# iqbal-lab-org/make_prg

Hardware: AMD Instinct MI355X
Metric: MSAs/sec (from_msa, whole node) on 30k-gene pan-genome (higher is better)
Workload: dtype u8 (+f64 KMeans)

## Files before the change

make_prg_amd/csrc/k_cluster.inc:

```
#define CF_TILE 256
#define CF_TILE_BIG 32
#define CF_ROWS 1024
static_assert(CF_TILE == MPRG_CF_TILE && CF_TILE_BIG == MPRG_CF_TILE_BIG && CF_ROWS == MPRG_CF_ROWS, "include/mprg.h documents the tiles");
MPRG_DEV long long cf_col_tiles(long long n_cols, long long n_rows) {
  const long long tw = n_rows > CF_ROWS ? CF_TILE_BIG : CF_TILE;
  return (n_cols + tw - 1) / tw;
}
#ifndef CFH_WIDE
#define CFH_WIDE MPRG_CF_WIDE
#endif
#define CFH_G 16
#define CFH_ROWS_WIDE 16
static_assert(CFH_ROWS_WIDE == MPRG_CF_ROWS_WIDE, "include/mprg.h documents the chunks");
MPRG_DEV int cf_chunk_rows(long long n_cols, long long n_rows) { return (n_cols >= CFH_WIDE && n_rows > CF_ROWS) ? CFH_ROWS_WIDE : CF_TILE; }
MPRG_DEV long long cf_row_chunks(long long n_cols, long long n_rows) { const int ch = cf_chunk_rows(n_cols, n_rows); return (n_rows + ch - 1) / ch; }
#define CFO_THREADS 128
#define CFO_POOL 8192
MPRG_DEV long long cf_lds_bytes(long long S, long long n, long long k) {
  const long long cp = (n + 3) & ~3LL;
  return ((S + 3) & ~3LL) + ((2 * S + 3) & ~3LL) + k * cp + S * cp;
}
MPRG_DEV bool cf_one_fits(long long S, long long n, long long k) { return S >= 1 && S < 65536 && n >= 1 && cf_lds_bytes(S, n, k) <= CFO_POOL; }
#ifndef CF_THREADS
#define CF_THREADS 128
#endif
KERNEL(k_cluster_majority, const uint8_t *arena, const int64_t *views, const int32_t *rowidx, const int64_t *prob_all,
       const int32_t *work, int k, const int32_t *d_of_row_all, const int32_t *labels_all, int32_t *assign_all,
       const double *km_info, int32_t *scratch_all, const uint8_t *gcodes_all, const int32_t *kinfo, int one_form, DsCount dc) {
  DS_GUARD(dc, 1);
  const int32_t *wk = work + 2 * (long long)BLOCK_ID;
  if (kinfo && kinfo[5 * (long long)wk[0] + 1] == 0) return;
  const int64_t *P = prob_all + (long long)wk[0] * PF;
  const ViewD d = load_view(views, (int)P[0]);
  if (one_form && cf_one_fits(d.n_rows, d.n_cols, k)) return;
  const int n = d.n_cols, S = d.n_rows, D = (int)P[1], tile = S > CF_ROWS ? CF_TILE_BIG : CF_TILE, c0 = wk[1] * tile;
  const int32_t *dor = d_of_row_all + d.row_off;
  const int32_t *labels = labels_all ? labels_all + P[10] : nullptr;
  uint8_t *maj = (uint8_t *)(scratch_all + d.col_off * 3);
  SHARED(uint32_t, cnt, 12 * CF_THREADS);
  SHARED(int32_t, first, 12 * CF_THREADS);
  if (wk[1] == 0 && labels && assign_all && (!km_info || km_info[8 * (long long)wk[0] + 3] >= (double)k)) {
    PAR_FOR(q, D) { assign_all[P[10] + q] = labels[q]; }
  }
  if (S > CF_ROWS) return;
  SHARED(int32_t, mrk, 2 * CF_ROWS);
  int32_t *mrow = mrk, *mkey = mrk + CF_ROWS;
  SHARED(int, coff, 16);
  SHARED(int, cfill, 16);
  PAR_FOR(q, 16) { coff[q] = 0; }
  BARRIER();
  PAR_FOR(i, S) {
    const int dd = dor[i];
    if (dd < 0) continue;
    const int cl = labels ? labels[dd] : 0;
    if (cl >= 0 && cl < k) ATOMIC_ADD(coff + cl + 1, 1);
  }
  BARRIER();
  ONE_THREAD { for (int q = 1; q <= k; ++q) coff[q] += coff[q - 1]; for (int q = 0; q < k; ++q) cfill[q] = coff[q]; }
  BARRIER();
  PAR_FOR(i, S) {
    const int dd = dor[i];
    if (dd < 0) continue;
    const int cl = labels ? labels[dd] : 0;
    if (cl < 0 || cl >= k) continue;
    const int pos = ATOMIC_ADD(cfill + cl, 1);
    mrow[pos] = gcodes_all ? (int)i : view_row(d, rowidx, i);
    mkey[pos] = dd * S + i;
  }
  BARRIER();
#define CF_COUNT(x, key) do { if ((x) < 12) { cnt[(x) * CF_THREADS + t] += 1; if ((key) < first[(x) * CF_THREADS + t]) first[(x) * CF_THREADS + t] = (key); } } while (0)
  const int ncols = n - c0 < tile ? n - c0 : tile;
  const int n_items = k * ncols;
  int slices = n_items <= N_THREADS ? N_THREADS / n_items : 1;
  if (slices > 8) slices = 8;
  for (int item0 = 0; item0 < n_items; item0 += N_THREADS) {
    const int t = (int)threadIdx.x;
    const int item = item0 + (slices > 1 ? t % n_items : t), sl = slices > 1 ? t / n_items : 0;
    const bool live = item < n_items && sl < slices;
    const int cl = live ? (int)((unsigned)item / (unsigned)ncols) : 0, c = c0 + (live ? (int)((unsigned)item % (unsigned)ncols) : 0);
    if (live) {
      for (int s = 0; s < 12; ++s) { cnt[s * CF_THREADS + t] = 0; first[s * CF_THREADS + t] = 0x7fffffff; }
      const uint8_t *col = gcodes_all ? gcodes_all + d.aux0 + c : arena + d.rm + d.col0 + c;
      const long long cpitch = gcodes_all ? u_pitch(n) : d.pitchC;
      const int lo = coff[cl], len = coff[cl + 1] - lo, per = (len + slices - 1) / slices;
      int m = lo + sl * per;
      const int m1 = lo + ((sl + 1) * per < len ? (sl + 1) * per : len);
      for (; m + 8 <= m1; m += 8) {
        unsigned x[8];
#pragma unroll
        for (int q = 0; q < 8; ++q) x[q] = col[(long long)mrow[m + q] * cpitch] & 15u;
#pragma unroll
        for (int q = 0; q < 8; ++q) CF_COUNT(x[q], mkey[m + q]);
      }
      for (; m < m1; ++m) { const unsigned x = col[(long long)mrow[m] * cpitch] & 15u; CF_COUNT(x, mkey[m]); }
    }
    if (slices > 1) BARRIER();
    if (live && sl == 0) {
      int best = 0; uint32_t best_n = 0; int32_t best_key = 0x7fffffff;
      for (int s = 0; s < 12; ++s) {
        uint32_t a = cnt[s * CF_THREADS + t]; int32_t key = first[s * CF_THREADS + t];
        for (int o = 1; o < slices; ++o) {
          a += cnt[s * CF_THREADS + t + o * n_items];
          const int32_t ko = first[s * CF_THREADS + t + o * n_items];
          if (ko < key) key = ko;
        }
        if (s == 0 || a > best_n || (a == best_n && key < best_key)) { best = s; best_n = a; best_key = key; }
      }
      maj[(long long)cl * n + c] = (uint8_t)best;
    }
  }
#undef CF_COUNT
}

#define CFB_THREADS 1024
KERNEL(k_cluster_majority_big, const uint8_t *arena, const int64_t *views, const int32_t *rowidx, const int64_t *prob_all,
       const int32_t *work, int k, const int32_t *d_of_row_all, const int32_t *labels_all, int32_t *scratch_all,
       const uint8_t *gcodes_all, const int32_t *kinfo, DsCount dc) {
  DS_GUARD(dc, 1);
  const int32_t *wk = work + 2 * (long long)BLOCK_ID;
  if (kinfo && kinfo[5 * (long long)wk[0] + 1] == 0) return;
  const int64_t *P = prob_all + (long long)wk[0] * PF;
  const ViewD d = load_view(views, (int)P[0]);
  const int n = d.n_cols, S = d.n_rows, c0 = wk[1] * CF_TILE_BIG;
  if (S <= CF_ROWS) return;
  const int32_t *dor = d_of_row_all + d.row_off;
  const int32_t *labels = labels_all ? labels_all + P[10] : nullptr;
  uint8_t *maj = (uint8_t *)(scratch_all + d.col_off * 3);
  __shared__ uint32_t cnt[KM_KMAX * CF_TILE_BIG * 12];
  __shared__ unsigned long long key[KM_KMAX * CF_TILE_BIG * 12];
  const int ncols = n - c0 < CF_TILE_BIG ? n - c0 : CF_TILE_BIG;
  PAR_FOR(e, k * CF_TILE_BIG * 12) { cnt[e] = 0; key[e] = ~0ULL; }
  BARRIER();
  const int t = (int)threadIdx.x, cg = t % (CF_TILE_BIG / 4), sl = t / (CF_TILE_BIG / 4), slices = N_THREADS / (CF_TILE_BIG / 4), cb = 4 * cg;
  if (cb < ncols && sl < slices) {
    const uint8_t *col = gcodes_all ? gcodes_all + d.aux0 + c0 + cb : arena + d.rm + d.col0 + c0 + cb;
    const long long cpitch = gcodes_all ? u_pitch(n) : d.pitchC;
    const int per = (S + slices - 1) / slices, i0 = sl * per, i1 = (sl + 1) * per < S ? (sl + 1) * per : S;
#define CFB_ROW(w_, dd_, i_, cl_) do {                                                                                                \
      const unsigned long long key_ = ((unsigned long long)(uint32_t)(dd_) << 32) | (uint32_t)(i_);                                   \
      _Pragma("unroll") for (int u_ = 0; u_ < 4; ++u_) {                                                                              \
        const unsigned x_ = ((w_) >> (8 * u_)) & 15u;                                                                                 \
        if (cb + u_ < ncols && x_ < 12) {                                                                                             \
          const int at_ = (((cl_) * CF_TILE_BIG + cb + u_) * 12) + (int)x_;                                                           \
          atomicAdd(&cnt[at_], 1u);                                                                                                   \
          if (key_ < key[at_]) atomicMin(&key[at_], key_);                                                                            \
        } } } while (0)
    int i = i0;
    for (; i + 8 <= i1; i += 8) {
      int dd8[8], lab8[8]; uint32_t w8[8];
#pragma unroll
      for (int q = 0; q < 8; ++q) dd8[q] = dor[i + q];
#pragma unroll
      for (int q = 0; q < 8; ++q) {
        lab8[q] = (labels && dd8[q] >= 0) ? labels[dd8[q]] : 0;
        __builtin_memcpy(&w8[q], col + (long long)(gcodes_all ? i + q : view_row(d, rowidx, i + q)) * cpitch, 4);
      }
#pragma unroll
      for (int q = 0; q < 8; ++q) if (dd8[q] >= 0 && lab8[q] >= 0 && lab8[q] < k) CFB_ROW(w8[q], dd8[q], i + q, lab8[q]);
    }
    for (; i < i1; ++i) {
      const int dd = dor[i];
      if (dd < 0) continue;
      const int cl = labels ? labels[dd] : 0;
      if (cl < 0 || cl >= k) continue;
// ... 175 lines not shown
```

make_prg_amd/csrc/k_kloop.inc:

```

#ifndef KL_CF_FN
#define KL_CF_FN MPRG_DEV
#endif
#ifdef MPRG_TEST_CF_GLOBAL
#define KL_CF_IN_LDS(fits) false
#else
#define KL_CF_IN_LDS(fits) (fits)
#endif
#define KL_CF_FIELD_BITS 32
MPRG_DEV int cf_row_cluster(int i, const uint8_t *mlab_s, const int32_t *dor, const int32_t *labels) {
  if (mlab_s) return mlab_s[i];
  const int dd = dor[i];
  return dd < 0 ? 255 : labels[dd];
}
template <int FB> struct CfWords {
  static constexpr int PER = 64 / FB, W = 12 / PER;
  unsigned long long w[W];
  MPRG_DEVM void clear() {
#pragma unroll
    for (int q = 0; q < W; ++q) w[q] = 0;
  }
  MPRG_DEVM void add(unsigned x) {
    const unsigned long long inc = x < 12 ? 1ull << (FB * (x % PER)) : 0ull;
    const unsigned sel = x / PER;
#pragma unroll
    for (int q = 0; q < W; ++q) w[q] += sel == (unsigned)q ? inc : 0ull;
  }
  MPRG_DEVM unsigned long long count(int s) const {
    return (w[s / PER] >> (FB * (s % PER))) & ((FB == 32) ? 0xffffffffull : 0xffffull);
  }
};
template <int FB, int POOLB>
KL_CF_FN bool cf_problem_fb(const int S, const int n, const int D, const int k, const int32_t *dor, const int32_t *labels, int32_t *assign,
                            uint8_t *maj, const uint8_t *G, uint8_t *pool, int *flag_s) {
  typedef CfWords<FB> Words;
  const int cpitch = u_pitch(n);
  const bool staged = S <= POOLB;
  uint8_t *mlab_w = staged ? pool : nullptr;
  const uint8_t *mlab_s = mlab_w;
  const int items = k * n;
  const long long acc_off = staged ? ((S + 7) & ~7) : 0;
  int slices = 1;
#ifndef KL_NO_SLICES
  if (items * 2 <= N_THREADS) {
    slices = N_THREADS / items; if (slices > 16) slices = 16;
    if (acc_off + (long long)items * slices * Words::W * 8 > POOLB) slices = 1;
  }
#endif
  unsigned long long *acc = (unsigned long long *)(pool + acc_off);
  PAR_FOR(q, D) { assign[q] = labels[q]; }
  if (staged) { PAR_FOR(i, S) { const int dd = dor[i]; mlab_w[i] = dd < 0 ? (uint8_t)255 : (uint8_t)labels[dd]; } }
  ONE_THREAD { flag_s[0] = 0; }
  BARRIER();
  for (int e0 = 0; e0 < items * slices; e0 += N_THREADS) {
    const int e = e0 + (int)threadIdx.x;
    const bool live = e < items * slices;
    const int item = live ? (slices > 1 ? e % items : e) : 0, sl = slices > 1 ? e / items : 0;
    const int cl = (int)((unsigned)item / (unsigned)n), c = (int)((unsigned)item % (unsigned)n);
    Words cw;
    cw.clear();
    const uint8_t *col = G + c;
    if (live) {
      const int per = (S + slices - 1) / slices;
      int i = sl * per;
      const int i1 = (sl + 1) * per < S ? (sl + 1) * per : S;
      for (; i + 4 <= i1; i += 4) {
        int rc[4]; unsigned x[4];
#pragma unroll
        for (int q = 0; q < 4; ++q) rc[q] = cf_row_cluster(i + q, mlab_s, dor, labels);
#pragma unroll
        for (int q = 0; q < 4; ++q) x[q] = rc[q] == cl ? (unsigned)col[(long long)(i + q) * cpitch] & 15u : 15u;
#pragma unroll
        for (int q = 0; q < 4; ++q) cw.add(x[q]);
      }
      for (; i < i1; ++i) if (cf_row_cluster(i, mlab_s, dor, labels) == cl) cw.add((unsigned)col[(long long)i * cpitch] & 15u);
      if (slices > 1 && sl > 0) {
#pragma unroll
        for (int q = 0; q < Words::W; ++q) acc[((long long)sl * items + item) * Words::W + q] = cw.w[q];
      }
    }
    if (slices > 1) {
      BARRIER();
      if (live && sl == 0) {
        for (int o = 1; o < slices; ++o)
#pragma unroll
          for (int q = 0; q < Words::W; ++q) cw.w[q] += acc[((long long)o * items + item) * Words::W + q];
      }
    }
    if (live && sl == 0) {
      unsigned long long best_n = 0;
#pragma unroll
      for (int s = 0; s < 12; ++s) { const unsigned long long a = cw.count(s); best_n = a > best_n ? a : best_n; }
      unsigned tied = 0;
#pragma unroll
      for (int s = 0; s < 12; ++s) if (cw.count(s) == best_n) tied |= 1u << s;
      int best = __ffs(tied) - 1;
      if (best_n > 0 && (tied & (tied - 1))) {
        long long best_key = 0x7fffffffffffffffLL;
#pragma nounroll
        for (int i = 0; i < S; ++i) {
          if (cf_row_cluster(i, mlab_s, dor, labels) != cl) continue;
          const unsigned x = (unsigned)col[(long long)i * cpitch] & 15u;
          if (!((tied >> x) & 1u)) continue;
          const long long key = (long long)dor[i] * S + i;
          if (key < best_key) { best_key = key; best = (int)x; }
        }
      }
      maj[(long long)cl * n + c] = (uint8_t)best;
    }
  }
  BARRIER();
  const int thresh = n < 5 ? 1 : (int)(0.2 * (double)n);
  PAR_FOR(i, S) {
    const int cl = cf_row_cluster((int)i, mlab_s, dor, labels);
    if (cl == 255) continue;
    const uint8_t *m = maj + (long long)cl * n;
    const uint8_t *grow = G + (long long)i * cpitch;
    int dist = 0;
#pragma nounroll
    for (int c = 0; c < n && dist <= thresh; c += 8) {
      uint64_t x, y;
      __builtin_memcpy(&x, grow + c, 8);
      __builtin_memcpy(&y, m + c, 8);
      uint64_t v = (x ^ y) & 0x0f0f0f0f0f0f0f0fULL;
      if (c + 8 > n) v &= 0xffffffffffffffffULL >> (8 * (c + 8 - n));
      const uint64_t nz = (((v & 0x7f7f7f7f7f7f7f7fULL) + 0x7f7f7f7f7f7f7f7fULL) | v) & 0x8080808080808080ULL;
      dist += __popcll(nz);
    }
    if (dist > thresh) flag_s[0] = 1;
  }
  BARRIER();
  const bool further = flag_s[0] != 0;
  BARRIER();
  return further;
}

template <bool OPT = false>
MPRG_DEV bool cf_problem_lds(const int S, const int n, const int D, const int k, const int32_t *dor, const int32_t *labels, int32_t *assign,
                             const uint8_t *G, uint8_t *pool, int *flag_s) {
  typedef CfWords<16> Words;
  const int cpitch = u_pitch(n), cp = (n + 3) & ~3, cw4 = cp >> 2;
  uint8_t *mlab = pool;
  uint16_t *dk = (uint16_t *)(pool + ((S + 3) & ~3));
  uint8_t *majs = (uint8_t *)dk + ((2 * S + 3) & ~3);
  uint8_t *cells = majs + k * cp;
  if (!OPT || assign) { PAR_FOR(q, D) { assign[q] = labels[q]; } }
  PAR_FOR(i, S) { const int dd = dor[i]; mlab[i] = dd < 0 ? (uint8_t)255 : ((OPT && !labels) ? (uint8_t)0 : (uint8_t)labels[dd]); dk[i] = (uint16_t)dd; }
  PAR_FOR(e, S * cw4) {
    const int i = (int)((unsigned)e / (unsigned)cw4), w = (int)((unsigned)e % (unsigned)cw4);
    *(uint32_t *)(cells + i * cp + 4 * w) = *(const uint32_t *)(G + (long long)i * cpitch + 4 * w) & 0x0f0f0f0fu;
  }
  ONE_THREAD { flag_s[0] = 0; }
  BARRIER();
  PAR_FOR(item, k * n) {
    const int cl = (int)((unsigned)item / (unsigned)n), c = (int)((unsigned)item % (unsigned)n);
    Words cw;
    cw.clear();
    const uint8_t *col = cells + c;
    int i = 0;
    for (; i + 4 <= S; i += 4) {
      unsigned rc[4], x[4];
#pragma unroll
      for (int q = 0; q < 4; ++q) { rc[q] = mlab[i + q]; x[q] = col[(i + q) * cp]; }
#pragma unroll
      for (int q = 0; q < 4; ++q) cw.add(rc[q] == (unsigned)cl ? x[q] : 15u);
    }
    for (; i < S; ++i) cw.add(mlab[i] == cl ? (unsigned)col[i * cp] : 15u);
    unsigned long long best_n = 0;
#pragma unroll
    for (int s_ = 0; s_ < 12; ++s_) { const unsigned long long a = cw.count(s_); best_n = a > best_n ? a : best_n; }
    unsigned tied = 0;
#pragma unroll
    for (int s_ = 0; s_ < 12; ++s_) if (cw.count(s_) == best_n) tied |= 1u << s_;
    int best = __ffs(tied) - 1;
    if (best_n > 0 && (tied & (tied - 1))) {
      int best_key = 0x7fffffff;
#pragma nounroll
      for (int r = 0; r < S; ++r) {
        const unsigned x = col[r * cp];
        if (mlab[r] != cl || !((tied >> x) & 1u)) continue;
        const int key = (int)dk[r] * S + r;
        if (key < best_key) { best_key = key; best = (int)x; }
      }
    }
    majs[cl * cp + c] = (uint8_t)best;
  }
  BARRIER();
  const int thresh = n < 5 ? 1 : (int)(0.2 * (double)n);
  PAR_FOR(i, S) {
    const int cl = mlab[i];
    if (cl == 255) continue;
    const uint8_t *m = majs + cl * cp, *row = cells + i * cp;
    int dist = 0;
#pragma nounroll
    for (int c = 0; c < n; c += 4) {
      uint32_t v = *(const uint32_t *)(row + c) ^ *(const uint32_t *)(m + c);
      if (c + 4 > n) v &= 0xffffffffu >> (8 * (c + 4 - n));
      const uint32_t nz = (((v & 0x7f7f7f7fu) + 0x7f7f7f7fu) | v) & 0x80808080u;
      dist += __popc(nz);
    }
    if (dist > thresh) flag_s[0] = 1;
  }
  BARRIER();
  const bool further = flag_s[0] != 0;
  BARRIER();
  return further;
}

struct KlUoff { int32_t v[KM_KMAX + 1]; };
enum { KL_ST_FITS = 80, KL_ST_BAD = 82, KL_ST_CF = 84, KL_ST_BYTES_GENERAL = 85, KL_ST_BYTES_SMALL = 93 };
template <int RMAX, int NEEDCAP, int LAB8, int POOLB, int KCH, int K_HI>
MPRG_DEV void kl_problem(const int b, const int64_t *prob_all, int n_init, const double *uniforms_all, const KlUoff &uoff,
                         const double *xcounts, double *ws_all, const int64_t *views, const int32_t *d_of_row_all,
                         const uint8_t *gcodes_all, int32_t *scratch_all, int32_t *labels_all, int32_t *assign_all, double *km_info,
                         int32_t *km_status, int32_t *num_clusters, int32_t *active, int64_t *stats, int bytes_slot, uint8_t *pool,
                         int sel_lab_cap) {
  SHARED(int32_t, ki_s, 8);
  SHARED(int, cf_flag, 1);
  SHARED(int, st_i, 4);
  SHARED(double, st_d, 2);
  ONE_THREAD { st_i[0] = num_clusters[b]; st_i[1] = 1; st_i[2] = 0; st_i[3] = 0; st_d[0] = 0; st_d[1] = 0; }
  BARRIER();
  for (;;) {
    const int k = st_i[0] + 1;
    const int D = (int)prob_all[(long long)b * PF + 1];
    BARRIER();
    if (k > KM_KMAX || k == D) { ONE_THREAD { st_i[0] = k; st_i[1] = 0; } break; }
    if (k > K_HI) break;
    ONE_THREAD { ki_s[0] = b; ki_s[1] = k; ki_s[2] = 0; ki_s[3] = uoff.v[k]; ki_s[4] = 0; km_status[b] = 0; }
    BARRIER();
    km_restarts_body<RMAX, NEEDCAP, LAB8, POOLB, KCH>(0, prob_all, ki_s, n_init, uniforms_all, xcounts, ws_all, nullptr, km_status + b, pool);
    BARRIER();
    KM_T0();
    km_select_body(0, prob_all, ki_s, n_init, xcounts, ws_all, nullptr, labels_all, km_info + 8 * (long long)b, (int32_t *)pool, sel_lab_cap);
    BARRIER(); KM_T(12);
    const int64_t *P = prob_all + (long long)b * PF;
    const double *info = km_info + 8 * (long long)b;
    const bool accepted = info[3] >= (double)k;
    const ViewD d = load_view(views, (int)P[0]);
    ONE_THREAD {
      st_i[2] += 1;
      st_d[0] += 8.0 * (double)P[1] * (double)P[7] * (info[4] + (double)n_init);
      if (km_status[b] & MPRG_KM_UNSUPPORTED) st_i[3] = 1;
      if (accepted) { st_i[0] = k; st_d[1] += (double)d.n_rows * (double)d.n_cols; }
      else st_i[1] = 0;
// ... 88 lines not shown
    BARRIER();
    KM_T0();
    const double *info = km_info + 8 * (long long)b;
    const bool accepted = info[3] >= (double)k;
    const ViewD d = load_view(views, (int)P[0]);
    ONE_THREAD {
      st_i[2] += 1;
      st_d[0] += 8.0 * (double)P[1] * (double)P[7] * (info[4] + (double)ki_s[5]);
      if (km_status[b] & MPRG_KM_UNSUPPORTED) st_i[3] = 1;
      if (accepted) { st_i[0] = k; st_d[1] += (double)d.n_rows * (double)d.n_cols; }
      else st_i[1] = 0;
    }
    if (!accepted) break;
    const int32_t *dor = d_of_row_all + d.row_off;
    int32_t *labels = labels_all + P[10], *assign = assign_all + P[10];
    uint8_t *maj = (uint8_t *)(scratch_all + d.col_off * 3);
    const uint8_t *G = gcodes_all + d.aux0;
    const bool cf_behind = KL_CF_IN_LDS(cf_lds_bytes(d.n_rows, d.n_cols, k) <= lds_size - head);
    const bool further = cf_behind ? cf_problem_lds(d.n_rows, d.n_cols, D, k, dor, labels, assign, G, pool + head, cf_flag)
                                   : cf_problem_fb<KL_CF_FIELD_BITS, KML_C0>(d.n_rows, d.n_cols, D, k, dor, labels, assign, maj, G, pool, cf_flag);
    if (!cf_behind) staged = false;
    KM_T(13);
    if (!further) { ONE_THREAD { st_i[1] = 0; } break; }
  }
  BARRIER();
  ONE_THREAD {
    num_clusters[b] = st_i[0]; active[b] = st_i[1];
    if (st_i[2]) {
      atomicAdd((unsigned long long *)stats + KL_ST_FITS, (unsigned long long)st_i[2]);
      atomicAdd((double *)stats + KL_ST_BYTES_SMALL, st_d[0]);
      if (st_d[1] != 0) atomicAdd((double *)stats + KL_ST_CF, st_d[1]);
      if (st_i[3]) stats[KL_ST_BAD] = 1;
    }
  }
}
__attribute__((amdgpu_flat_work_group_size(64, 1024), amdgpu_waves_per_eu(KM_WAVES, KM_WAVES))) __global__ void k_cluster_loop_lds(
    const int64_t *prob_all, int n_init, const double *uniforms_all, KlUoff uoff, const double *xcounts, double *ws_all,
    const int64_t *views, const int32_t *d_of_row_all, const uint8_t *gcodes_all, int32_t *scratch_all, int32_t *labels_all,
    int32_t *assign_all, double *km_info, int32_t *km_status, int32_t *num_clusters, int32_t *active, int64_t *stats, int cls, int lds_bytes,
    DsCount dc) {
  DS_GUARD(dc, 1);
  HIP_DYNAMIC_SHARED(uint8_t, pool)
  const int b = BLOCK_ID;
  if (!active[b]) return;
  const int64_t *P = prob_all + (long long)b * PF;
  const int c = kml_class_ws(P[1], P[7], num_clusters[b] + 1, n_init, true, ws_all + P[9]);
  if (c < 0 || c > cls) return;
  kll_problem(b, prob_all, n_init, uniforms_all, uoff, xcounts, ws_all, views, d_of_row_all, gcodes_all, scratch_all, labels_all, assign_all, km_info,
              km_status, num_clusters, active, stats, pool, lds_bytes, cls);
}

KERNEL(k_cluster_further_one, const int64_t *views, const int64_t *prob_all, int n_probs, int k, const int32_t *d_of_row_all,
       const int32_t *labels_all, int32_t *assign_all, const double *km_info, int32_t *out_further, const uint8_t *gcodes_all,
       const int32_t *kinfo, DsCount dc) {
  DS_GUARD(dc, 1);
  const int b = BLOCK_ID;
  if (kinfo && kinfo[5 * (long long)b + 1] == 0) return;
  const int64_t *P = prob_all + (long long)b * PF;
  const ViewD d = load_view(views, (int)P[0]);
  if (!cf_one_fits(d.n_rows, d.n_cols, k)) return;
  __shared__ __attribute__((aligned(16))) uint8_t pool[CFO_POOL];
  SHARED(int, flag, 1);
  const int32_t *labels = labels_all ? labels_all + P[10] : nullptr;
  int32_t *assign = (labels && assign_all && (!km_info || km_info[8 * (long long)b + 3] >= (double)k)) ? assign_all + P[10] : nullptr;
  const bool further = cf_problem_lds<true>(d.n_rows, d.n_cols, (int)P[1], k, d_of_row_all + d.row_off, labels, assign, gcodes_all + d.aux0, pool, flag);
  ONE_THREAD { out_further[b] = further ? 1 : 0; }
}
```

make_prg_amd/csrc/mprg_api.hip:

```cpp
#include "mprg_platform.h"
#include "../../include/mprg.h"
#include <stdio.h>
#include <initializer_list>
#include <string.h>

#include "k_ingest.inc"
#include "k_columns.inc"
#include "k_partition.inc"
#include "k_rows.inc"
#include "k_kmer.inc"
#include "k_kmeans.inc"
#include "k_kmeans_lds.inc"
#include "k_cluster.inc"
#include "k_kloop.inc"
#include "k_emit.inc"
#include "k_forest.inc"
#include "k_align.inc"
#include "k_star.inc"
#include "k_refine.inc"
#include "k_prog.inc"
#include "k_prog_band.inc"
#include "k_collapse.inc"
#include "host_encoders.inc"
#include "host_batch.inc"

static thread_local char g_err[512] = "";
static int fail(const char *what) { snprintf(g_err, sizeof g_err, "%s", what); return -1; }

static int check_launch(const char *name) {
  hipError_t e = hipGetLastError();
  if (e != hipSuccess) { snprintf(g_err, sizeof g_err, "%s: %s", name, hipGetErrorString(e)); return -2; }
  return 0;
}

#include "runtime_api.inc"

#define BLOCK_VIEW 256
#include <stdlib.h>
static int env_threads(const char *name, int dflt, int hi = 1024) {
  const char *e = getenv(name);
  const int v = e ? atoi(e) : dflt;
  return (v >= 64 && v <= hi && v % 64 == 0) ? v : dflt;
}
static const int g_pf_threads = env_threads("MPRG_PF_THREADS", BLOCK_VIEW);
static const int g_dd_threads = env_threads("MPRG_DD_THREADS", BLOCK_VIEW, 512);
static const int g_km_threads = env_threads("MPRG_KM_THREADS", 256);
static const int g_km_wide_threads = env_threads("MPRG_KM_WIDE_THREADS", 1024);
static const int g_kp_threads = env_threads("MPRG_KP_THREADS", 0);
static const int g_kp_tiled = [] { const char *e = getenv("MPRG_KP_TILED"); return (e && atoi(e) == 0) ? 0 : 1; }();
static const int g_kpw_split = [] { const char *e = getenv("MPRG_KPW_SPLIT"); return (e && atoi(e) == 0) ? 0 : 1; }();
static const int g_kms_threads = env_threads("MPRG_KMS_THREADS", 128, 128);
static const int g_kml_flags = [] { const char *e = getenv("MPRG_KML_FLAGS"); return e ? (atoi(e) & 0x7f) : 0; }();
static const int g_kml_threads[KML_CLASSES] = {env_threads("MPRG_KML_THREADS0", 128, 256), env_threads("MPRG_KML_THREADS1", 128, 256),
                                               env_threads("MPRG_KML_THREADS2", 256, 1024), env_threads("MPRG_KML_THREADS3", 256, 1024),
                                               env_threads("MPRG_KML_THREADS4", 512, 1024), env_threads("MPRG_KML_THREADS5", 1024, 1024)};
template <class K> static int kml_raise_lds(K kernel, bool *raised, const char *what) {
  if (*raised) return 0;
  if (hipFuncSetAttribute((const void *)kernel, hipFuncAttributeMaxDynamicSharedMemorySize, KML_C5) != hipSuccess) return fail(what);
  *raised = true;
  return 0;
}
static const int g_cf_one = [] { const char *e = getenv("MPRG_CF_ONE"); return (e && atoi(e) == 0) ? 0 : 1; }();
static const int g_pw_wave = [] { const char *e = getenv("MPRG_WAVE_VIEWS"); return (e && atoi(e) == 0) ? 0 : 1; }();
static const int g_row_views = [] { const char *e = getenv("MPRG_ROW_VIEWS"); return (e && atoi(e) == 0) ? 0 : 1; }();
#define RV_THREADS 128
#define RV_THREADS_S 64

extern "C" {

#ifndef MPRG_BUILD_TAG
#define MPRG_BUILD_TAG "hip gfx950"
#endif
const char *mprg_version(void) { return "mprg 0.2 (" MPRG_BUILD_TAG ")"; }
const char *mprg_last_error(void) { return g_err; }

int mprg_device_cus(void) {
  int dev = 0; hipDeviceProp_t p;
  if (hipGetDevice(&dev) != hipSuccess || hipGetDeviceProperties(&p, dev) != hipSuccess) return fail("no HIP device");
  return p.multiProcessorCount;
}

int mprg_ingest(const uint8_t *raw, const int64_t *msa_table, int n_msas, int64_t n_tiles, const uint8_t *n_replacement,
                uint8_t *arena, int64_t arena_bytes, int32_t *status, void *stream) {
  if (n_msas <= 0) return 0;
  if (hipMemsetAsync(arena, 15, (size_t)arena_bytes, (hipStream_t)stream) != hipSuccess) return fail("memset");
  if (hipMemsetAsync(status, 0, sizeof(int32_t) * n_msas, (hipStream_t)stream) != hipSuccess) return fail("memset");
  if (n_tiles > 0) LAUNCH(k_ingest, n_tiles, 256, stream, raw, msa_table, n_msas, n_replacement, arena, status);
  return check_launch("k_ingest");
}

int mprg_column_residue_counts(const uint8_t *raw, const int64_t *table, const int32_t *work, int n_work, int32_t *out,
                               void *stream) {
  if (n_work <= 0) return 0;
  LAUNCH(k_column_residue_counts, n_work, 256, stream, raw, table, work, out);
  return check_launch("k_column_residue_counts");
}

static int d_column_masks(const uint8_t *arena, const int64_t *views, const int32_t *rowidx, const int32_t *work,
                          int n_items, int rows_per_chunk, uint32_t *out_mask, void *stream, DsCount dc) {
  if (n_items <= 0) return 0;
  if (rows_per_chunk <= 0) return fail("rows_per_chunk must be positive");
  LAUNCH(k_column_masks, n_items, CM_THREADS, stream, arena, views, rowidx, work, rows_per_chunk, out_mask, dc);
  return check_launch("k_column_masks");
}
int mprg_column_masks(const uint8_t *arena, const int64_t *views, const int32_t *rowidx, const int32_t *work,
                      int n_items, int rows_per_chunk, uint32_t *out_mask, void *stream) {
  return d_column_masks(arena, views, rowidx, work, n_items, rows_per_chunk, out_mask, stream, DS_HOST);
}

int mprg_compact_columns(const uint8_t *arena, const int64_t *views, const int32_t *rowidx, const int32_t *work, int n_items,
                         int rows_per_chunk, const uint32_t *mask, uint8_t *out, const int64_t *out_off, int32_t *kept, void *stream) {
  if (n_items <= 0) return 0;
  if (rows_per_chunk <= 0) return fail("rows_per_chunk must be positive");
  LAUNCH(k_compact_columns, n_items, CC_THREADS, stream, arena, views, rowidx, work, rows_per_chunk, mask, out, out_off, kept);
  return check_launch("k_compact_columns");
// ... 289 lines not shown

int mprg_kmeans_fit_lds(const int64_t *prob, const int32_t *kinfo, const int32_t *fit_list, int n_fits, int lds_class, int n_init,
                        const double *uniforms_dev, const double *xcounts, double *ws, int32_t *labels, double *km_info,
                        int32_t *km_status, void *stream) {
  if (n_fits <= 0) return 0;
  if (n_init < 1 || n_init > KML_RMAX) return fail("mprg_kmeans_fit_lds: n_init must be 1..10");
  if (lds_class < 0 || lds_class >= KML_CLASSES) return fail("mprg_kmeans_fit_lds: lds_class must be 0..5 (mprg_kmeans_lds_class)");
  const int bytes = kml_class_bytes(lds_class);
  static bool raised = false;
  if (bytes > 56 * 1024 && kml_raise_lds(k_kmeans_fit_lds, &raised, "mprg_kmeans_fit_lds: the device refuses the LDS of the largest class") != 0) return -1;
  LAUNCH_LDS(k_kmeans_fit_lds, n_fits, g_kml_threads[lds_class], bytes, stream, prob, kinfo, fit_list, n_init, uniforms_dev, xcounts, ws, labels,
             km_info, km_status, bytes | (g_kml_flags << 24));
  return check_launch("k_kmeans_fit_lds");
}

int mprg_kmeans_select(const int64_t *prob, const int32_t *kinfo, int n_fits, int n_init, const double *xcounts,
                       double *ws, int32_t *labels, double *km_info, void *stream) {
  if (n_fits <= 0) return 0;
  LAUNCH(k_kmeans_select, n_fits, 256, stream, prob, kinfo, n_init, xcounts, ws, labels, km_info);
  return check_launch("k_kmeans_select");
}

static int d_cluster_further(const uint8_t *arena, const int64_t *views, const int32_t *rowidx, const int64_t *prob,
                             int n_probs, int k, const int32_t *d_of_row, const int32_t *labels, int32_t *assign,
                             const int32_t *work_cols, int n_work_cols, const int32_t *work_rows, int n_work_rows,
                             int32_t *scratch, int32_t *out_further, const double *km_info, const uint8_t *gcodes, const int32_t *kinfo,
                             void *stream, DsCount dc_cols, DsCount dc_rows, DsCount dc_probs, long long max_rows = 0);
int mprg_cluster_further(const uint8_t *arena, const int64_t *views, const int32_t *rowidx, const int64_t *prob,
                         int n_probs, int k, const int32_t *d_of_row, const int32_t *labels, int32_t *assign,
                         const int32_t *work_cols, int n_work_cols, const int32_t *work_rows, int n_work_rows,
                         int32_t *scratch, int32_t *out_further, const double *km_info, const uint8_t *gcodes, const int32_t *kinfo,
                         void *stream) {
  return d_cluster_further(arena, views, rowidx, prob, n_probs, k, d_of_row, labels, assign, work_cols, n_work_cols, work_rows, n_work_rows,
                           scratch, out_further, km_info, gcodes, kinfo, stream, DS_HOST, DS_HOST, DS_HOST);
}
int mprg_cluster_further_bounded(const uint8_t *arena, const int64_t *views, const int32_t *rowidx, const int64_t *prob,
                                 int n_probs, int k, const int32_t *d_of_row, const int32_t *labels, int32_t *assign,
                                 const int32_t *work_cols, int n_work_cols, const int32_t *work_rows, int n_work_rows,
                                 int32_t *scratch, int32_t *out_further, const double *km_info, const uint8_t *gcodes, const int32_t *kinfo,
                                 long long max_rows, void *stream) {
  return d_cluster_further(arena, views, rowidx, prob, n_probs, k, d_of_row, labels, assign, work_cols, n_work_cols, work_rows, n_work_rows,
                           scratch, out_further, km_info, gcodes, kinfo, stream, DS_HOST, DS_HOST, DS_HOST, max_rows);
}
static int d_cluster_further(const uint8_t *arena, const int64_t *views, const int32_t *rowidx, const int64_t *prob,
                             int n_probs, int k, const int32_t *d_of_row, const int32_t *labels, int32_t *assign,
                             const int32_t *work_cols, int n_work_cols, const int32_t *work_rows, int n_work_rows,
                             int32_t *scratch, int32_t *out_further, const double *km_info, const uint8_t *gcodes, const int32_t *kinfo,
                             void *stream, DsCount dc_cols, DsCount dc_rows, DsCount dc_probs, long long max_rows) {
  if (n_probs <= 0) return 0;
  if (k < 1 || k > KM_KMAX) return fail("mprg_cluster_further: k out of range");
  if (hipMemsetAsync(out_further, 0, sizeof(int32_t) * n_probs, (hipStream_t)stream) != hipSuccess) return fail("memset");
  const int one = (g_cf_one && gcodes) ? 1 : 0;
  if (one) LAUNCH(k_cluster_further_one, n_probs, CFO_THREADS, stream, views, prob, n_probs, k, d_of_row, labels, assign, km_info, out_further, gcodes,
                  kinfo, dc_probs);
  const int big = (max_rows <= 0 || max_rows > CF_ROWS) ? 1 : 0;
  LAUNCH(k_cluster_majority, n_work_cols, CF_THREADS, stream, arena, views, rowidx, prob, work_cols, k, d_of_row, labels,
         assign, km_info, scratch, gcodes, kinfo, one, dc_cols);
  if (big) LAUNCH(k_cluster_majority_big, n_work_cols, CFB_THREADS, stream, arena, views, rowidx, prob, work_cols, k, d_of_row, labels,
                  scratch, gcodes, kinfo, dc_cols);
  LAUNCH(k_cluster_hamming, n_work_rows, CF_TILE, stream, arena, views, rowidx, prob, work_rows, d_of_row, labels,
         (const int32_t *)scratch, out_further, gcodes, kinfo, one ? k : 0, dc_rows);
  return check_launch("k_cluster_further");
}

static int d_cluster_loop(const int64_t *views, const int64_t *prob, int n_probs, int n_init, const double *uniforms_dev,
                          const int32_t *uniform_offsets_host, const double *xcounts, double *ws, const int32_t *d_of_row,
                          const uint8_t *gcodes, int32_t *scratch, int32_t *labels, int32_t *assign, double *km_info, int32_t *km_status,
                          int32_t *num_clusters, int32_t *active, int64_t *stats, int forms, void *stream, DsCount dc);
int mprg_cluster_loop(const int64_t *views, const int64_t *prob, int n_probs, int n_init, const double *uniforms_dev,
                      const int32_t *uniform_offsets_host, const double *xcounts, double *ws, const int32_t *d_of_row,
                      const uint8_t *gcodes, int32_t *scratch, int32_t *labels, int32_t *assign, double *km_info, int32_t *km_status,
                      int32_t *num_clusters, int32_t *active, int64_t *stats, int forms, void *stream) {
  return d_cluster_loop(views, prob, n_probs, n_init, uniforms_dev, uniform_offsets_host, xcounts, ws, d_of_row, gcodes, scratch, labels, assign,
                        km_info, km_status, num_clusters, active, stats, forms, stream, DS_HOST);
}
static int d_cluster_loop(const int64_t *views, const int64_t *prob, int n_probs, int n_init, const double *uniforms_dev,
                          const int32_t *uniform_offsets_host, const double *xcounts, double *ws, const int32_t *d_of_row,
                          const uint8_t *gcodes, int32_t *scratch, int32_t *labels, int32_t *assign, double *km_info, int32_t *km_status,
                          int32_t *num_clusters, int32_t *active, int64_t *stats, int forms, void *stream, DsCount dc) {
  if (n_probs <= 0) return 0;
  if (n_init < 1 || n_init > KM_RMAX) return fail("n_init must be 1..16");
  if (!gcodes || !uniform_offsets_host || !stats) return fail("mprg_cluster_loop: gcodes, uniform_offsets_host and stats are required");
  if (!(forms & (7 | MPRG_LOOP_LDS))) return fail("mprg_cluster_loop: forms must name a workgroup form (MPRG_LOOP_*)");
  KlUoff uoff;
  for (int k = 0; k <= KM_KMAX; ++k) uoff.v[k] = k >= 2 ? uniform_offsets_host[k] : 0;
  const bool small_ok = n_init <= KMS_RMAX;
  static bool raised_loop = false;
  if ((forms & MPRG_LOOP_LDS) && n_init <= KML_RMAX &&
      kml_raise_lds(k_cluster_loop_lds, &raised_loop, "mprg_cluster_loop: the device refuses the LDS of the largest class") != 0) return -1;
  if ((forms & MPRG_LOOP_LDS) && n_init <= KML_RMAX)
    for (int c = 0; c < KML_CLASSES; ++c)
      LAUNCH_LDS(k_cluster_loop_lds, n_probs, g_kml_threads[c], kml_class_bytes(c), stream, prob, n_init, uniforms_dev, uoff, xcounts, ws, views, d_of_row,
                 gcodes, scratch, labels, assign, km_info, km_status, num_clusters, active, stats, c, kml_class_bytes(c) | (g_kml_flags << 24), dc);
  if (forms & MPRG_LOOP_GENERAL)
    LAUNCH(k_cluster_loop, n_probs, g_km_threads, stream, prob, n_init, uniforms_dev, uoff, xcounts, ws, views, d_of_row, gcodes, scratch, labels,
           assign, km_info, km_status, num_clusters, active, stats,
           (((forms & MPRG_LOOP_SKIP_SMALL) && small_ok) ? 1 : 0) | (((forms & MPRG_LOOP_SKIP_LDS) && n_init <= KML_RMAX) ? 2 : 0), dc);
#define KLS_LAUNCH(KCH, KHI) hipLaunchKernelGGL((k_cluster_loop_small<KCH, KHI>), dim3((unsigned)n_probs), dim3(128), 0, (hipStream_t)stream, prob, \
                                                 n_init, uniforms_dev, uoff, xcounts, ws, views, d_of_row, gcodes, scratch, labels, assign, \
                                                 km_info, km_status, num_clusters, active, stats, dc)
  if ((forms & MPRG_LOOP_SMALL_LOW) && small_ok) KLS_LAUNCH(36, 6);
  if ((forms & MPRG_LOOP_SMALL_HIGH) && small_ok) KLS_LAUNCH(KM_KMAX * KM_KMAX, KM_KMAX);
#undef KLS_LAUNCH
  return check_launch("k_cluster_loop");
}

int mprg_split_children(const int64_t *views, const int32_t *rowidx, const int64_t *prob, int n_probs,
                        const int64_t *split_info, const int32_t *d_of_row, const int32_t *s_of_row,
                        const int32_t *assign, int32_t *pool_out, int32_t *child_sizes, void *stream) {
  if (n_probs <= 0) return 0;
// ... 629 lines not shown
```

Baseline: 135,100.

## Bucket rows by cluster and count majority votes in packed registers

Adds a cluster-bucketed variant of the single-block cluster-further path. Rows are ranked per cluster with wave ballots and their cells are copied contiguously into LDS. The majority kernel now keeps per-symbol counts in packed 16-bit register words, reduces them across slices with lane shuffles, and resolves ties in a second pass only when one occurs. This removes the LDS count and first-key arrays and the per-element shared-memory updates, at the cost of a rescan on ties and a slightly larger LDS pool budget. The old paths stay available behind an environment flag.

Result: faster. 137,100 (median of 5 runs) (+1.5%).

```diff
diff --git a/make_prg_amd/csrc/k_cluster.inc b/make_prg_amd/csrc/k_cluster.inc
--- a/make_prg_amd/csrc/k_cluster.inc
+++ b/make_prg_amd/csrc/k_cluster.inc
@@ -15,19 +15,36 @@
 MPRG_DEV int cf_chunk_rows(long long n_cols, long long n_rows) { return (n_cols >= CFH_WIDE && n_rows > CF_ROWS) ? CFH_ROWS_WIDE : CF_TILE; }
 MPRG_DEV long long cf_row_chunks(long long n_cols, long long n_rows) { const int ch = cf_chunk_rows(n_cols, n_rows); return (n_rows + ch - 1) / ch; }
 #define CFO_THREADS 128
-#define CFO_POOL 8192
+#define CFO_POOL 8448
 MPRG_DEV long long cf_lds_bytes(long long S, long long n, long long k) {
   const long long cp = (n + 3) & ~3LL;
-  return ((S + 3) & ~3LL) + ((2 * S + 3) & ~3LL) + k * cp + S * cp;
+  return 2 * ((2 * S + 3) & ~3LL) + k * cp + S * cp;
 }
 MPRG_DEV bool cf_one_fits(long long S, long long n, long long k) { return S >= 1 && S < 65536 && n >= 1 && cf_lds_bytes(S, n, k) <= CFO_POOL; }
 #ifndef CF_THREADS
 #define CF_THREADS 128
 #endif
-KERNEL(k_cluster_majority, const uint8_t *arena, const int64_t *views, const int32_t *rowidx, const int64_t *prob_all,
-       const int32_t *work, int k, const int32_t *d_of_row_all, const int32_t *labels_all, int32_t *assign_all,
-       const double *km_info, int32_t *scratch_all, const uint8_t *gcodes_all, const int32_t *kinfo, int one_form, DsCount dc) {
-  DS_GUARD(dc, 1);
+template <int FB> struct CfWords {
+  static constexpr int PER = 64 / FB, W = 12 / PER;
+  unsigned long long w[W];
+  MPRG_DEVM void clear() {
+#pragma unroll
+    for (int q = 0; q < W; ++q) w[q] = 0;
+  }
+  MPRG_DEVM void add(unsigned x) {
+    const unsigned long long inc = x < 12 ? 1ull << (FB * (x % PER)) : 0ull;
+    const unsigned sel = x / PER;
+#pragma unroll
+    for (int q = 0; q < W; ++q) w[q] += sel == (unsigned)q ? inc : 0ull;
+  }
+  MPRG_DEVM unsigned long long count(int s) const {
+    return (w[s / PER] >> (FB * (s % PER))) & ((FB == 32) ? 0xffffffffull : 0xffffull);
+  }
+};
+template <bool REGS>
+MPRG_DEV void cf_majority_tile(const uint8_t *arena, const int64_t *views, const int32_t *rowidx, const int64_t *prob_all,
+                               const int32_t *work, int k, const int32_t *d_of_row_all, const int32_t *labels_all, int32_t *assign_all,
+                               const double *km_info, int32_t *scratch_all, const uint8_t *gcodes_all, const int32_t *kinfo, int one_form) {
   const int32_t *wk = work + 2 * (long long)BLOCK_ID;
   if (kinfo && kinfo[5 * (long long)wk[0] + 1] == 0) return;
   const int64_t *P = prob_all + (long long)wk[0] * PF;
@@ -37,8 +54,6 @@
   const int32_t *dor = d_of_row_all + d.row_off;
   const int32_t *labels = labels_all ? labels_all + P[10] : nullptr;
   uint8_t *maj = (uint8_t *)(scratch_all + d.col_off * 3);
-  SHARED(uint32_t, cnt, 12 * CF_THREADS);
-  SHARED(int32_t, first, 12 * CF_THREADS);
   if (wk[1] == 0 && labels && assign_all && (!km_info || km_info[8 * (long long)wk[0] + 3] >= (double)k)) {
     PAR_FOR(q, D) { assign_all[P[10] + q] = labels[q]; }
   }
@@ -68,48 +83,114 @@
     mkey[pos] = dd * S + i;
   }
   BARRIER();
-#define CF_COUNT(x, key) do { if ((x) < 12) { cnt[(x) * CF_THREADS + t] += 1; if ((key) < first[(x) * CF_THREADS + t]) first[(x) * CF_THREADS + t] = (key); } } while (0)
   const int ncols = n - c0 < tile ? n - c0 : tile;
   const int n_items = k * ncols;
-  int slices = n_items <= N_THREADS ? N_THREADS / n_items : 1;
-  if (slices > 8) slices = 8;
-  for (int item0 = 0; item0 < n_items; item0 += N_THREADS) {
-    const int t = (int)threadIdx.x;
-    const int item = item0 + (slices > 1 ? t % n_items : t), sl = slices > 1 ? t / n_items : 0;
-    const bool live = item < n_items && sl < slices;
-    const int cl = live ? (int)((unsigned)item / (unsigned)ncols) : 0, c = c0 + (live ? (int)((unsigned)item % (unsigned)ncols) : 0);
-    if (live) {
-      for (int s = 0; s < 12; ++s) { cnt[s * CF_THREADS + t] = 0; first[s * CF_THREADS + t] = 0x7fffffff; }
-      const uint8_t *col = gcodes_all ? gcodes_all + d.aux0 + c : arena + d.rm + d.col0 + c;
-      const long long cpitch = gcodes_all ? u_pitch(n) : d.pitchC;
-      const int lo = coff[cl], len = coff[cl + 1] - lo, per = (len + slices - 1) / slices;
-      int m = lo + sl * per;
-      const int m1 = lo + ((sl + 1) * per < len ? (sl + 1) * per : len);
+  const uint8_t *cells = gcodes_all ? gcodes_all + d.aux0 : arena + d.rm + d.col0;
+  const long long cpitch = gcodes_all ? u_pitch(n) : d.pitchC;
+  if constexpr (REGS) {
+    typedef CfWords<16> Words;
+    int sh = 0;
+    while (sh < 3 && (n_items << (sh + 1)) <= N_THREADS) ++sh;
+    const int slices = 1 << sh;
+    for (int e0 = 0; e0 < (n_items << sh); e0 += N_THREADS) {
+      const int e = e0 + (int)threadIdx.x;
+      const bool live = e < (n_items << sh);
+      const int item = live ? e >> sh : 0, sl = e & (slices - 1);
+      const int cl = (int)((unsigned)item / (unsigned)ncols), c = c0 + (int)((unsigned)item % (unsigned)ncols);
+      const uint8_t *col = cells + c;
+      const int lo = coff[cl], len = live ? coff[cl + 1] - lo : 0, per = (len + slices - 1) >> sh;
+      const int m0 = lo + (sl * per < len ? sl * per : len), m1 = lo + ((sl + 1) * per < len ? (sl + 1) * per : len);
+      Words cw;
+      cw.clear();
+      int m = m0;
       for (; m + 8 <= m1; m += 8) {
         unsigned x[8];
 #pragma unroll
         for (int q = 0; q < 8; ++q) x[q] = col[(long long)mrow[m + q] * cpitch] & 15u;
 #pragma unroll
-        for (int q = 0; q < 8; ++q) CF_COUNT(x[q], mkey[m + q]);
-      }
-      for (; m < m1; ++m) { const unsigned x = col[(long long)mrow[m] * cpitch] & 15u; CF_COUNT(x, mkey[m]); }
-    }
-    if (slices > 1) BARRIER();
-    if (live && sl == 0) {
-      int best = 0; uint32_t best_n = 0; int32_t best_key = 0x7fffffff;
-      for (int s = 0; s < 12; ++s) {
-        uint32_t a = cnt[s * CF_THREADS + t]; int32_t key = first[s * CF_THREADS + t];
-        for (int o = 1; o < slices; ++o) {
-          a += cnt[s * CF_THREADS + t + o * n_items];
-          const int32_t ko = first[s * CF_THREADS + t + o * n_items];
-          if (ko < key) key = ko;
+        for (int q = 0; q < 8; ++q) cw.add(x[q]);
+      }
+      for (; m < m1; ++m) cw.add(col[(long long)mrow[m] * cpitch] & 15u);
+      for (int dl = 1; dl < slices; dl <<= 1) {
+#pragma unroll
+        for (int q = 0; q < Words::W; ++q) cw.w[q] += __shfl_xor(cw.w[q], dl);
+      }
+      unsigned long long best_n = 0;
+#pragma unroll
+      for (int s = 0; s < 12; ++s) { const unsigned long long a = cw.count(s); best_n = a > best_n ? a : best_n; }
+      unsigned tied = 0;
+#pragma unroll
+      for (int s = 0; s < 12; ++s) if (cw.count(s) == best_n) tied |= 1u << s;
+      int best = __ffs(tied) - 1;
+      unsigned pick = 0xffffffffu;
+      if (best_n > 0 && (tied & (tied - 1))) {
+#pragma nounroll
+        for (m = m0; m < m1; ++m) {
+          const unsigned x = col[(long long)mrow[m] * cpitch] & 15u;
+          if (!((tied >> x) & 1u)) continue;
+          const unsigned key = ((unsigned)mkey[m] << 4) | x;
+          pick = key < pick ? key : pick;
         }
-        if (s == 0 || a > best_n || (a == best_n && key < best_key)) { best = s; best_n = a; best_key = key; }
-      }
-      maj[(long long)cl * n + c] = (uint8_t)best;
-    }
-  }
+      }
+      for (int dl = 1; dl < slices; dl <<= 1) { const unsigned o = __shfl_xor(pick, dl); pick = o < pick ? o : pick; }
+      if (pick != 0xffffffffu) best = (int)(pick & 15u);
+      if (live && sl == 0) maj[(long long)cl * n + c] = (uint8_t)best;
+    }
+  } else {
+    SHARED(uint32_t, cnt, 12 * CF_THREADS);
+    SHARED(int32_t, first, 12 * CF_THREADS);
+#define CF_COUNT(x, key) do { if ((x) < 12) { cnt[(x) * CF_THREADS + t] += 1; if ((key) < first[(x) * CF_THREADS + t]) first[(x) * CF_THREADS + t] = (key); } } while (0)
+    int slices = n_items <= N_THREADS ? N_THREADS / n_items : 1;
+    if (slices > 8) slices = 8;
+    for (int item0 = 0; item0 < n_items; item0 += N_THREADS) {
+      const int t = (int)threadIdx.x;
+      const int item = item0 + (slices > 1 ? t % n_items : t), sl = slices > 1 ? t / n_items : 0;
+      const bool live = item < n_items && sl < slices;
+      const int cl = live ? (int)((unsigned)item / (unsigned)ncols) : 0, c = c0 + (live ? (int)((unsigned)item % (unsigned)ncols) : 0);
+      if (live) {
+        for (int s = 0; s < 12; ++s) { cnt[s * CF_THREADS + t] = 0; first[s * CF_THREADS + t] = 0x7fffffff; }
+        const uint8_t *col = cells + c;
+        const int lo = coff[cl], len = coff[cl + 1] - lo, per = (len + slices - 1) / slices;
+        int m = lo + sl * per;
+        const int m1 = lo + ((sl + 1) * per < len ? (sl + 1) * per : len);
+        for (; m + 8 <= m1; m += 8) {
+          unsigned x[8];
+#pragma unroll
+          for (int q = 0; q < 8; ++q) x[q] = col[(long long)mrow[m + q] * cpitch] & 15u;
+#pragma unroll
+          for (int q = 0; q < 8; ++q) CF_COUNT(x[q], mkey[m + q]);
+        }
+        for (; m < m1; ++m) { const unsigned x = col[(long long)mrow[m] * cpitch] & 15u; CF_COUNT(x, mkey[m]); }
+      }
+      if (slices > 1) BARRIER();
+      if (live && sl == 0) {
+        int best = 0; uint32_t best_n = 0; int32_t best_key = 0x7fffffff;
+        for (int s = 0; s < 12; ++s) {
+          uint32_t a = cnt[s * CF_THREADS + t]; int32_t key = first[s * CF_THREADS + t];
+          for (int o = 1; o < slices; ++o) {
+            a += cnt[s * CF_THREADS + t + o * n_items];
+            const int32_t ko = first[s * CF_THREADS + t + o * n_items];
+            if (ko < key) key = ko;
+          }
+          if (s == 0 || a > best_n || (a == best_n && key < best_key)) { best = s; best_n = a; best_key = key; }
+        }
+        maj[(long long)cl * n + c] = (uint8_t)best;
+      }
+    }
 #undef CF_COUNT
+  }
+}
+KERNEL(k_cluster_majority, const uint8_t *arena, const int64_t *views, const int32_t *rowidx, const int64_t *prob_all,
+       const int32_t *work, int k, const int32_t *d_of_row_all, const int32_t *labels_all, int32_t *assign_all,
+       const double *km_info, int32_t *scratch_all, const uint8_t *gcodes_all, const int32_t *kinfo, int one_form, DsCount dc) {
+  DS_GUARD(dc, 1);
+  cf_majority_tile<true>(arena, views, rowidx, prob_all, work, k, d_of_row_all, labels_all, assign_all, km_info, scratch_all, gcodes_all, kinfo, one_form);
+}
+KERNEL(k_cluster_majority_lds, const uint8_t *arena, const int64_t *views, const int32_t *rowidx, const int64_t *prob_all,
+       const int32_t *work, int k, const int32_t *d_of_row_all, const int32_t *labels_all, int32_t *assign_all,
+       const double *km_info, int32_t *scratch_all, const uint8_t *gcodes_all, const int32_t *kinfo, int one_form, DsCount dc) {
+  DS_GUARD(dc, 1);
+  cf_majority_tile<false>(arena, views, rowidx, prob_all, work, k, d_of_row_all, labels_all, assign_all, km_info, scratch_all, gcodes_all, kinfo, one_form);
 }
 
 #define CFB_THREADS 1024
diff --git a/make_prg_amd/csrc/k_kloop.inc b/make_prg_amd/csrc/k_kloop.inc
--- a/make_prg_amd/csrc/k_kloop.inc
+++ b/make_prg_amd/csrc/k_kloop.inc
@@ -13,23 +13,6 @@
   const int dd = dor[i];
   return dd < 0 ? 255 : labels[dd];
 }
-template <int FB> struct CfWords {
-  static constexpr int PER = 64 / FB, W = 12 / PER;
-  unsigned long long w[W];
-  MPRG_DEVM void clear() {
-#pragma unroll
-    for (int q = 0; q < W; ++q) w[q] = 0;
-  }
-  MPRG_DEVM void add(unsigned x) {
-    const unsigned long long inc = x < 12 ? 1ull << (FB * (x % PER)) : 0ull;
-    const unsigned sel = x / PER;
-#pragma unroll
-    for (int q = 0; q < W; ++q) w[q] += sel == (unsigned)q ? inc : 0ull;
-  }
-  MPRG_DEVM unsigned long long count(int s) const {
-    return (w[s / PER] >> (FB * (s % PER))) & ((FB == 32) ? 0xffffffffull : 0xffffull);
-  }
-};
 template <int FB, int POOLB>
 KL_CF_FN bool cf_problem_fb(const int S, const int n, const int D, const int k, const int32_t *dor, const int32_t *labels, int32_t *assign,
                             uint8_t *maj, const uint8_t *G, uint8_t *pool, int *flag_s) {
@@ -136,7 +119,7 @@
 }
 
 template <bool OPT = false>
-MPRG_DEV bool cf_problem_lds(const int S, const int n, const int D, const int k, const int32_t *dor, const int32_t *labels, int32_t *assign,
+MPRG_DEV bool cf_problem_lds_rows(const int S, const int n, const int D, const int k, const int32_t *dor, const int32_t *labels, int32_t *assign,
                              const uint8_t *G, uint8_t *pool, int *flag_s) {
   typedef CfWords<16> Words;
   const int cpitch = u_pitch(n), cp = (n + 3) & ~3, cw4 = cp >> 2;
@@ -191,6 +174,128 @@
     const int cl = mlab[i];
     if (cl == 255) continue;
     const uint8_t *m = majs + cl * cp, *row = cells + i * cp;
+    int dist = 0;
+#pragma nounroll
+    for (int c = 0; c < n; c += 4) {
+      uint32_t v = *(const uint32_t *)(row + c) ^ *(const uint32_t *)(m + c);
+      if (c + 4 > n) v &= 0xffffffffu >> (8 * (c + 4 - n));
+      const uint32_t nz = (((v & 0x7f7f7f7fu) + 0x7f7f7f7fu) | v) & 0x80808080u;
+      dist += __popc(nz);
+    }
+    if (dist > thresh) flag_s[0] = 1;
+  }
+  BARRIER();
+  const bool further = flag_s[0] != 0;
+  BARRIER();
+  return further;
+}
+
+template <bool OPT = false>
+MPRG_DEV bool cf_problem_lds(const int S, const int n, const int D, const int k, const int32_t *dor, const int32_t *labels, int32_t *assign,
+                             const uint8_t *G, uint8_t *pool, int *flag_s) {
+  typedef CfWords<16> Words;
+  SHARED(int, off, 12);
+  const int cpitch = u_pitch(n), cp = (n + 3) & ~3, cw4 = cp >> 2;
+  uint16_t *pos = (uint16_t *)pool;
+  uint16_t *dk = (uint16_t *)(pool + ((2 * S + 3) & ~3));
+  uint8_t *majs = (uint8_t *)dk + ((2 * S + 3) & ~3);
+  uint8_t *cells = majs + k * cp;
+  uint8_t *lab = cells;
+  if (!OPT || assign) { PAR_FOR(q, D) { assign[q] = labels[q]; } }
+  PAR_FOR(i, S) {
+    const int dd = dor[i];
+    const int cl = dd < 0 ? 255 : ((OPT && !labels) ? 0 : labels[dd]);
+    lab[i] = (unsigned)cl < (unsigned)k ? (uint8_t)cl : (uint8_t)255;
+  }
+  ONE_THREAD { flag_s[0] = 0; }
+  BARRIER();
+  if (MPRG_TID < WAVE) {
+    const int lane = MPRG_TID;
+    const unsigned long long below = (1ull << lane) - 1ull;
+    int run = 0;
+    for (int i0 = 0; i0 < S; i0 += WAVE) {
+      const int i = i0 + lane;
+      const int cl = i < S ? (int)lab[i] : 255;
+      const int before = run;
+      int rank = 0;
+      for (int q = 0; q < k; ++q) {
+        const unsigned long long m = __ballot(cl == q);
+        if (cl == q) rank = __popcll(m & below);
+        if (lane == q) run += __popcll(m);
+      }
+      const int base = __shfl(before, cl < k ? cl : 0);
+      if (cl < k) pos[i] = (uint16_t)(base + rank);
+    }
+    const int incl = wave_scan_incl(run);
+    if (lane <= k) off[lane] = incl - run;
+  }
+  BARRIER();
+  PAR_FOR(i, S) {
+    const int cl = lab[i];
+    if (cl == 255) { pos[i] = (uint16_t)0xffff; continue; }
+    const int p = off[cl] + (int)pos[i];
+    pos[i] = (uint16_t)p; dk[p] = (uint16_t)dor[i];
+  }
+  BARRIER();
+  const int M = off[k];
+  PAR_FOR(e, S * cw4) {
+    const int i = (int)((unsigned)e / (unsigned)cw4), w = (int)((unsigned)e % (unsigned)cw4), p = pos[i];
+    if (p != 0xffff) *(uint32_t *)(cells + p * cp + 4 * w) = *(const uint32_t *)(G + (long long)i * cpitch + 4 * w) & 0x0f0f0f0fu;
+  }
+  BARRIER();
+  const int items = k * n;
+  int sh = 0;
+  while (sh < 4 && (items << (sh + 1)) <= N_THREADS) ++sh;
+  const int slices = 1 << sh;
+  for (int e0 = 0; e0 < (items << sh); e0 += N_THREADS) {
+    const int e = e0 + MPRG_TID;
+    const bool live = e < (items << sh);
+    const int item = live ? e >> sh : 0, sl = e & (slices - 1);
+    const int cl = (int)((unsigned)item / (unsigned)n), c = (int)((unsigned)item % (unsigned)n);
+    const int lo = off[cl], len = live ? off[cl + 1] - lo : 0, per = (len + slices - 1) >> sh;
+    const int p0 = lo + (sl * per < len ? sl * per : len), p1 = lo + ((sl + 1) * per < len ? (sl + 1) * per : len);
+    const uint8_t *col = cells + c;
+    Words cw;
+    cw.clear();
+    int p = p0;
+    for (; p + 4 <= p1; p += 4) {
+      unsigned x[4];
+#pragma unroll
+      for (int q = 0; q < 4; ++q) x[q] = col[(p + q) * cp];
+#pragma unroll
+      for (int q = 0; q < 4; ++q) cw.add(x[q]);
+    }
+    for (; p < p1; ++p) cw.add((unsigned)col[p * cp]);
+    for (int d = 1; d < slices; d <<= 1) {
+#pragma unroll
+      for (int q = 0; q < Words::W; ++q) cw.w[q] += __shfl_xor(cw.w[q], d);
+    }
+    unsigned long long best_n = 0;
+#pragma unroll
+    for (int s_ = 0; s_ < 12; ++s_) { const unsigned long long a = cw.count(s_); best_n = a > best_n ? a : best_n; }
+    unsigned tied = 0;
+#pragma unroll
+    for (int s_ = 0; s_ < 12; ++s_) if (cw.count(s_) == best_n) tied |= 1u << s_;
+    int best = __ffs(tied) - 1;
+    unsigned pick = 0xffffffffu;
+    if (best_n > 0 && (tied & (tied - 1))) {
+#pragma nounroll
+      for (int r = p0; r < p1; ++r) {
+        if (!((tied >> col[r * cp]) & 1u)) continue;
+        const unsigned key = ((unsigned)dk[r] << 16) | (unsigned)r;
+        pick = key < pick ? key : pick;
+      }
+    }
+    for (int d = 1; d < slices; d <<= 1) { const unsigned o = __shfl_xor(pick, d); pick = o < pick ? o : pick; }
+    if (pick != 0xffffffffu) best = (int)col[(pick & 0xffffu) * cp];
+    if (live && sl == 0) majs[cl * cp + c] = (uint8_t)best;
+  }
+  BARRIER();
+  const int thresh = n < 5 ? 1 : (int)(0.2 * (double)n);
+  PAR_FOR(p, M) {
+    int cl = 0;
+    for (int q = 1; q < k; ++q) cl += (int)p >= off[q] ? 1 : 0;
+    const uint8_t *m = majs + cl * cp, *row = cells + p * cp;
     int dist = 0;
 #pragma nounroll
     for (int c = 0; c < n; c += 4) {
@@ -385,7 +490,7 @@
 
 KERNEL(k_cluster_further_one, const int64_t *views, const int64_t *prob_all, int n_probs, int k, const int32_t *d_of_row_all,
        const int32_t *labels_all, int32_t *assign_all, const double *km_info, int32_t *out_further, const uint8_t *gcodes_all,
-       const int32_t *kinfo, DsCount dc) {
+       const int32_t *kinfo, int buckets, DsCount dc) {
   DS_GUARD(dc, 1);
   const int b = BLOCK_ID;
   if (kinfo && kinfo[5 * (long long)b + 1] == 0) return;
@@ -396,6 +501,7 @@
   SHARED(int, flag, 1);
   const int32_t *labels = labels_all ? labels_all + P[10] : nullptr;
   int32_t *assign = (labels && assign_all && (!km_info || km_info[8 * (long long)b + 3] >= (double)k)) ? assign_all + P[10] : nullptr;
-  const bool further = cf_problem_lds<true>(d.n_rows, d.n_cols, (int)P[1], k, d_of_row_all + d.row_off, labels, assign, gcodes_all + d.aux0, pool, flag);
+  const bool further = buckets ? cf_problem_lds<true>(d.n_rows, d.n_cols, (int)P[1], k, d_of_row_all + d.row_off, labels, assign, gcodes_all + d.aux0, pool, flag)
+                               : cf_problem_lds_rows<true>(d.n_rows, d.n_cols, (int)P[1], k, d_of_row_all + d.row_off, labels, assign, gcodes_all + d.aux0, pool, flag);
   ONE_THREAD { out_further[b] = further ? 1 : 0; }
 }
diff --git a/make_prg_amd/csrc/mprg_api.hip b/make_prg_amd/csrc/mprg_api.hip
--- a/make_prg_amd/csrc/mprg_api.hip
+++ b/make_prg_amd/csrc/mprg_api.hip
@@ -61,6 +61,7 @@
   return 0;
 }
 static const int g_cf_one = [] { const char *e = getenv("MPRG_CF_ONE"); return (e && atoi(e) == 0) ? 0 : 1; }();
+static const int g_cf_buckets = [] { const char *e = getenv("MPRG_CF_BUCKETS"); return (e && atoi(e) == 0) ? 0 : 1; }();
 static const int g_pw_wave = [] { const char *e = getenv("MPRG_WAVE_VIEWS"); return (e && atoi(e) == 0) ? 0 : 1; }();
 static const int g_row_views = [] { const char *e = getenv("MPRG_ROW_VIEWS"); return (e && atoi(e) == 0) ? 0 : 1; }();
 #define RV_THREADS 128
@@ -456,10 +457,12 @@
   if (hipMemsetAsync(out_further, 0, sizeof(int32_t) * n_probs, (hipStream_t)stream) != hipSuccess) return fail("memset");
   const int one = (g_cf_one && gcodes) ? 1 : 0;
   if (one) LAUNCH(k_cluster_further_one, n_probs, CFO_THREADS, stream, views, prob, n_probs, k, d_of_row, labels, assign, km_info, out_further, gcodes,
-                  kinfo, dc_probs);
+                  kinfo, g_cf_buckets, dc_probs);
   const int big = (max_rows <= 0 || max_rows > CF_ROWS) ? 1 : 0;
-  LAUNCH(k_cluster_majority, n_work_cols, CF_THREADS, stream, arena, views, rowidx, prob, work_cols, k, d_of_row, labels,
-         assign, km_info, scratch, gcodes, kinfo, one, dc_cols);
+  if (g_cf_buckets) LAUNCH(k_cluster_majority, n_work_cols, CF_THREADS, stream, arena, views, rowidx, prob, work_cols, k, d_of_row, labels,
+                           assign, km_info, scratch, gcodes, kinfo, one, dc_cols);
+  else LAUNCH(k_cluster_majority_lds, n_work_cols, CF_THREADS, stream, arena, views, rowidx, prob, work_cols, k, d_of_row, labels,
+              assign, km_info, scratch, gcodes, kinfo, one, dc_cols);
   if (big) LAUNCH(k_cluster_majority_big, n_work_cols, CFB_THREADS, stream, arena, views, rowidx, prob, work_cols, k, d_of_row, labels,
                   scratch, gcodes, kinfo, dc_cols);
   LAUNCH(k_cluster_hamming, n_work_rows, CF_TILE, stream, arena, views, rowidx, prob, work_rows, d_of_row, labels,
```
